# GenomicBreeding/GenomicBreedingModels.jl

Hardware: AMD Instinct MI355X
Metric: GRM+GBLUP genotype-cells/s (n x p) (higher is better)
Workload: dtype f64

## Files before the change

### genomicbreedingmodels.jl_amd/csrc/grm.hip

```cpp
#include <algorithm>
#include <atomic>
#include <cmath>
#include <cstdio>
#include <cstdlib>
#include <map>
#include <mutex>
#include <queue>
#include <tuple>
#include <vector>

#include "chol_device.h"

namespace gbm {

constexpr int BT = 128;
constexpr int BK = 16;
constexpr int WPS = 2;
constexpr int LROW = BT + 2;
constexpr int STAGE = 2 * BK * LROW;

__device__ __forceinline__ void tile_of(int64_t t, int64_t& ti, int64_t& tj) {
  int64_t r = (int64_t)((sqrt(8.0 * (double)t + 1.0) - 1.0) * 0.5);
  while ((r + 1) * (r + 2) / 2 <= t) r++;
  while (r * (r + 1) / 2 > t) r--;
  tj = r;
  ti = t - r * (r + 1) / 2;
}

enum SyrkMode { kSub = 0, kSplit = 1, kPersist = 2, kPersistFused = 3 };

struct TileOwner {
  int32_t rank = 0, nranks = 1;
  int64_t rhs_tile = -1;
  int64_t j_first = 0, ncols = 0;
  int32_t rhs = 0;
  int64_t ti0 = 0;
};

template <bool NEG>
__device__ __forceinline__ void tile_pass(const double* __restrict__ U, int64_t ldu, int64_t K, int64_t i0,
                                          int64_t j0, bool diag, bool active, int64_t kstep0, int64_t nsteps,
                                          double* lds, d4 (&acc)[4][4], int wave, int lane) {
  const int wm = wave >> 1, wn = wave & 1;
  auto stage_row = [&](int64_t kstep, int buf, int rr) {
    double* base = lds + buf * STAGE;
    const int r = wave * (BK / 4) + rr;
    const int64_t k = kstep * BK + r;
    double* la = base + r * LROW;
    double* lb = base + (BK + r) * LROW;
#ifdef GBM_SYRK_TIMING_NOLOAD
    if (k < K) {
    } else {
#else
    if (k < K) {
      const double* src = U + k * ldu;
      __builtin_amdgcn_global_load_lds((const void*)(src + i0 + lane * 2), (void*)la, 16, 0, 0);
      if (!diag) __builtin_amdgcn_global_load_lds((const void*)(src + j0 + lane * 2), (void*)lb, 16, 0, 0);
    } else {
#endif
      *reinterpret_cast<double2*>(la + lane * 2) = make_double2(0.0, 0.0);
      if (!diag) *reinterpret_cast<double2*>(lb + lane * 2) = make_double2(0.0, 0.0);
    }
  };
  const int frag_row = lane >> 4;
  const int frag_col = lane & 15;

  if (nsteps > 0) {
#pragma unroll
    for (int rr = 0; rr < BK / 4; rr++) stage_row(kstep0, 0, rr);
  }
  __syncthreads();
  for (int64_t st = 0; st < nsteps; st++) {
    const int buf = (int)(st & 1);
    if (st + 1 < nsteps) {
#pragma unroll
      for (int rr = 0; rr < BK / 4; rr++) stage_row(kstep0 + st + 1, buf ^ 1, rr);
    }
    const double* A = lds + buf * STAGE;
    const double* B = diag ? A : A + BK * LROW;
#pragma unroll
    for (int ks = 0; ks < BK / 4; ks++) {
      if (active) {
        const int kr = ks * 4 + frag_row;
        const double2 a01 = *reinterpret_cast<const double2*>(&A[kr * LROW + wm * 64 + 4 * frag_col]);
        const double2 a23 = *reinterpret_cast<const double2*>(&A[kr * LROW + wm * 64 + 4 * frag_col + 2]);
        const double2 b01 = *reinterpret_cast<const double2*>(&B[kr * LROW + wn * 64 + 4 * frag_col]);
        const double2 b23 = *reinterpret_cast<const double2*>(&B[kr * LROW + wn * 64 + 4 * frag_col + 2]);
        double af[4] = {a01.x, a01.y, a23.x, a23.y};
        const double bf[4] = {b01.x, b01.y, b23.x, b23.y};
        if constexpr (NEG) {
#pragma unroll
          for (int m = 0; m < 4; m++) af[m] = -af[m];
        }
        __builtin_amdgcn_s_setprio(1);
#pragma unroll
        for (int m = 0; m < 4; m++)
#pragma unroll
          for (int q = 0; q < 4; q++)
            acc[m][q] = __builtin_amdgcn_mfma_f64_16x16x4f64(af[m], bf[q], acc[m][q], 0, 0, 0);
        __builtin_amdgcn_s_setprio(0);
      }
    }
    __syncthreads();
  }
  __syncthreads();
}

constexpr int kMaxSlices = 32;
struct SliceBounds {
  int32_t n;
  int32_t b[kMaxSlices + 1];
  int32_t carry;
  int32_t er, et, erb, es, ekper;
  int64_t e0, eslab_off;
  int32_t accum = 0;
  int32_t fuse = 0;
};

template <int ET>
__device__ __forceinline__ void grm_edge_pass(const double* __restrict__ U, int64_t ldu, int64_t K,
                                              const SliceBounds& sb, int64_t e, double* __restrict__ part,
                                              int lane, int wave) {
  const int rb = (int)(e % sb.erb), ks = (int)(e / sb.erb);
  const int64_t k0 = (int64_t)ks * sb.ekper;
  const int64_t k1 = (k0 + sb.ekper < K) ? k0 + sb.ekper : K;
  const int64_t i0 = (int64_t)rb * 256 + wave * 64;
  const int fr = lane >> 4, fc = lane & 15;
  d4 acc[4][ET];
#pragma unroll
  for (int m = 0; m < 4; m++)
#pragma unroll
    for (int q = 0; q < ET; q++) acc[m][q] = (d4){0.0, 0.0, 0.0, 0.0};
  for (int64_t k = k0; k < k1; k += 16) {
    double a[4][4], b[4][ET];
#pragma unroll
    for (int st = 0; st < 4; st++) {
      const int64_t kk = k + st * 4 + fr;
      const bool kv = kk < k1;
      const double* row = U + kk * ldu;
#pragma unroll
      for (int m = 0; m < 4; m++) {
        const int64_t i = i0 + m * 16 + fc;
        a[st][m] = (kv && i < ldu) ? row[i] : 0.0;
      }
#pragma unroll
      for (int q = 0; q < ET; q++) b[st][q] = kv ? row[sb.e0 + q * 16 + fc] : 0.0;
    }
#pragma unroll
    for (int st = 0; st < 4; st++)
#pragma unroll
      for (int q = 0; q < ET; q++)
#pragma unroll
        for (int m = 0; m < 4; m++) acc[m][q] = __builtin_amdgcn_mfma_f64_16x16x4f64(a[st][m], b[st][q], acc[m][q], 0, 0, 0);
  }
  const int64_t rows = (int64_t)sb.erb * 256;
  constexpr int w = 16 * ET;
#pragma unroll
  for (int m = 0; m < 4; m++)
#pragma unroll
    for (int q = 0; q < ET; q++)
#pragma unroll
      for (int r = 0; r < 4; r++)
        part[((int64_t)ks * rows + i0 + m * 16 + fr + 4 * r) * w + q * 16 + fc] = acc[m][q][r];
}

template <int ET>
__global__ void __launch_bounds__(256, ET == 1 ? 4 : 1) grm_edge_kernel(const double* __restrict__ U, int64_t ldu, int64_t K,
                                                       SliceBounds sb, double* __restrict__ part) {
  grm_edge_pass<ET>(U, ldu, K, sb, blockIdx.x, part, threadIdx.x & 63, threadIdx.x >> 6);
}

__global__ void __launch_bounds__(256) grm_edge_reduce_kernel(const double* __restrict__ part, int64_t n,
                                                              SliceBounds sb, double* __restrict__ G, int64_t ldg,
                                                              int accum) {
  const int64_t idx = (int64_t)blockIdx.x * 256 + threadIdx.x;
  if (idx >= n * sb.er) return;
  const int64_t i = idx / sb.er;
  const int c = (int)(idx - i * sb.er);
  const int64_t rows = (int64_t)sb.erb * 256;
  const int w = 16 * sb.et;
  double acc = 0.0;
  for (int s = 0; s < sb.es; s++) acc += part[((int64_t)s * rows + i) * w + c];
  double* g = G + i * ldg + sb.e0 + c;
  *g = accum ? *g + acc : acc;
}

template <int MODE>
__global__ void __launch_bounds__(256, WPS)
syrk_kernel(const double* __restrict__ U, int64_t ldu, int64_t K, int64_t c0, int64_t lim,
            double* __restrict__ C, int64_t ldc, double* __restrict__ slab, int64_t ntiles, SliceBounds sb,
            double* __restrict__ Ld, double* __restrict__ Dinv, int32_t* __restrict__ info, int64_t fk0,
            TileOwner own) {
  constexpr int LDS_DOUBLES = (2 * STAGE > CNB * PS + CNB + 16) ? 2 * STAGE : CNB * PS + CNB + 16;
  __shared__ __attribute__((aligned(16))) double lds[LDS_DOUBLES];

  const int64_t wg = blockIdx.x;
  const int lane = threadIdx.x & 63;
  const int wave = __builtin_amdgcn_readfirstlane(threadIdx.x >> 6);
  const int wm = wave >> 1, wn = wave & 1;
  const int frag_row = lane >> 4, frag_col = lane & 15;
  const int64_t nst = (K + BK - 1) / BK;
  const int64_t rlim = c0 + lim;

  if constexpr (MODE == kSplit || MODE == kPersist || MODE == kPersistFused) {
    auto run_unit = [&](int sl, int64_t t) {
    int64_t ti, tj;
    tile_of(t, ti, tj);
    const bool diag = (ti == tj);
    const int64_t i0 = c0 + ti * BT, j0 = c0 + tj * BT;
    const bool active = (i0 + wm * 64 < rlim) && (j0 + wn * 64 < rlim) && !(diag && wm == 1 && wn == 0);
    d4 acc[4][4];
#pragma unroll
    for (int a = 0; a < 4; a++)
#pragma unroll
      for (int b = 0; b < 4; b++) acc[a][b] = (d4){0.0, 0.0, 0.0, 0.0};
    const int64_t ks0 = sb.b[sl];
    const int64_t ks1 = sb.b[sl + 1] < nst ? sb.b[sl + 1] : nst;
    tile_pass<false>(U, ldu, K, i0, j0, diag, active, ks0, ks1 > ks0 ? ks1 - ks0 : 0, lds, acc, wave, lane);
    if (MODE == kSplit && sb.carry && sb.n > 1) {
      int32_t* tflags = reinterpret_cast<int32_t*>(slab);
      double* out = C + i0 * ldc + j0 + (wm * 64 + 4 * frag_row) * ldc + wn * 64 + 4 * frag_col;
      if (sl > 0 || sb.accum) {
        if (sl > 0) {
          if (threadIdx.x == 0) wait_flag(&tflags[t], sl, tflags + ntiles);
          __syncthreads();
          __builtin_amdgcn_fence(__ATOMIC_ACQUIRE, "agent");
        }
        if (active) {
          double2 prev[4][4][2];
#pragma unroll
          for (int m = 0; m < 4; m++)
#pragma unroll
            for (int r = 0; r < 4; r++) {
              const double* o = out + (16 * r + m) * ldc;
              prev[m][r][0] = *reinterpret_cast<const double2*>(o);
              prev[m][r][1] = *reinterpret_cast<const double2*>(o + 2);
            }
#pragma unroll
          for (int m = 0; m < 4; m++)
#pragma unroll
            for (int r = 0; r < 4; r++) {
              acc[m][0][r] = prev[m][r][0].x + acc[m][0][r];
              acc[m][1][r] = prev[m][r][0].y + acc[m][1][r];
              acc[m][2][r] = prev[m][r][1].x + acc[m][2][r];
              acc[m][3][r] = prev[m][r][1].y + acc[m][3][r];
            }
        }
      }
      if (active) {
#pragma unroll
        for (int m = 0; m < 4; m++)
#pragma unroll
          for (int r = 0; r < 4; r++) {
            double* o = out + (16 * r + m) * ldc;
#pragma unroll
            for (int q = 0; q < 4; q++) st_agent(o + q, acc[m][q][r]);
          }
      }
      publish_flag(&tflags[t], sl + 1, threadIdx.x);
    } else if (MODE == kPersistFused && sb.n > 1) {
      const int64_t per = (int64_t)BT * BT;
      const int64_t eoff = (wm * 64 + 4 * frag_row) * BT + wn * 64 + 4 * frag_col;
      if (active) {
        double* out = slab + ((int64_t)sl * ntiles + t) * per + eoff;
#pragma unroll
        for (int m = 0; m < 4; m++)
#pragma unroll
          for (int r = 0; r < 4; r++) {
            double* o = out + (16 * r + m) * BT;
            *reinterpret_cast<double2*>(o) = make_double2(acc[m][0][r], acc[m][1][r]);
            *reinterpret_cast<double2*>(o + 2) = make_double2(acc[m][2][r], acc[m][3][r]);
          }
      }
      asm volatile("s_waitcnt vmcnt(0)" ::: "memory");
      __syncthreads();
      int* s_last = reinterpret_cast<int*>(lds);
      if (threadIdx.x == 0) {
        __builtin_amdgcn_fence(__ATOMIC_RELEASE, "agent");
        asm volatile("s_waitcnt vmcnt(0)" ::: "memory");
        const bool lt = __hip_atomic_fetch_add(&info[8 + t], 1, __ATOMIC_RELAXED, __HIP_MEMORY_SCOPE_AGENT) == sb.n - 1;
        if (lt) {
          __builtin_amdgcn_fence(__ATOMIC_ACQUIRE, "agent");
          asm volatile("s_waitcnt vmcnt(0)" ::: "memory");
        }
        *s_last = lt;
      }
      __syncthreads();
      const bool last = *s_last != 0;
      __syncthreads();
      if (last && active) {
        double* gout = C + (i0 + wm * 64 + 4 * frag_row) * ldc + j0 + wn * 64 + 4 * frag_col;
        const double* tbase = slab + t * per + eoff;
#pragma unroll 1
        for (int mr = 0; mr < 16; mr++) {
          const int m = mr & 3, r = mr >> 2;
          double2 v01 = make_double2(0.0, 0.0), v23 = make_double2(0.0, 0.0);
          for (int s2 = 0; s2 < sb.n; s2++) {
            const double* src = tbase + (int64_t)s2 * ntiles * per + (16 * r + m) * BT;
            const double2 x01 = *reinterpret_cast<const double2*>(src), x23 = *reinterpret_cast<const double2*>(src + 2);
            v01.x += x01.x;
            v01.y += x01.y;
            v23.x += x23.x;
            v23.y += x23.y;
          }
          double* g = gout + (16 * r + m) * ldc;
          if (sb.accum) {
            const double2 a01 = *reinterpret_cast<const double2*>(g), a23 = *reinterpret_cast<const double2*>(g + 2);
            v01 = make_double2(a01.x + v01.x, a01.y + v01.y);
            v23 = make_double2(a23.x + v23.x, a23.y + v23.y);
          }
          *reinterpret_cast<double2*>(g) = v01;
          *reinterpret_cast<double2*>(g + 2) = v23;
        }
      }
    } else if (active) {
      const int64_t ld = sb.n == 1 ? ldc : BT;
      double* out = (sb.n == 1 ? C + i0 * ldc + j0 : slab + ((int64_t)sl * ntiles + t) * (BT * BT)) +
                    (wm * 64 + 4 * frag_row) * ld + wn * 64 + 4 * frag_col;
#pragma unroll
      for (int m = 0; m < 4; m++)
#pragma unroll
        for (int r = 0; r < 4; r++) {
          double* o = out + (16 * r + m) * ld;
          *reinterpret_cast<double2*>(o) = make_double2(acc[m][0][r], acc[m][1][r]);
          *reinterpret_cast<double2*>(o + 2) = make_double2(acc[m][2][r], acc[m][3][r]);
        }
    }
    };
    const int64_t T8 = (ntiles + 7) & ~(int64_t)7;
    if constexpr (MODE == kPersist || MODE == kPersistFused) {
      __shared__ int64_t s_unit;
      int32_t* ctr = info;
      const int xcc = (int)(__builtin_amdgcn_s_getreg((20 << 0) | (0 << 6) | (31 << 11)) & 7);
      const int64_t per = T8 >> 3;
      int q = xcc;
      for (int tries = 0; tries < 8;) {
        const int64_t qt0 = q * per;
        const int64_t qt1 = qt0 + per < ntiles ? qt0 + per : ntiles;
        const int64_t nq = qt1 > qt0 ? qt1 - qt0 : 0;
        if (threadIdx.x == 0) s_unit = atomicAdd(&ctr[q], 1);
        __syncthreads();
        const int64_t u = s_unit;
        __syncthreads();
        if (u >= nq * sb.n) {
          q = (q + 1) & 7;
          tries++;
          continue;
        }
        const int sl = (int)(u / nq);
        run_unit(sl, qt0 + (u - (int64_t)sl * nq));
      }
      return;
    } else {
      const int sl = (int)(wg / T8);
      const int64_t u = wg - (int64_t)sl * T8;
      const int64_t t = (u & 7) * (T8 >> 3) + (u >> 3);
      if (t >= ntiles) return;
      run_unit(sl, t);
    }
    return;
  } else {
    int64_t ti, tj;
    if (own.nranks > 1) {
      const int64_t c = blockIdx.y;
      const int64_t J = c < own.ncols ? own.j_first + c * own.nranks : own.rhs_tile;
      tj = J - c0 / BT;
      ti = own.ti0 + blockIdx.x;
      if (ti > tj) return;
    } else {
      tile_of(wg, ti, tj);
    }
    const bool diag = (ti == tj);
    const int64_t i0 = c0 + ti * BT, j0 = c0 + tj * BT;
    const bool active = (i0 + wm * 64 < rlim) && (j0 + wn * 64 < rlim) && !(diag && wm == 1 && wn == 0);
    d4 acc[4][4];
    const int64_t col0 = j0 + wn * 64 + 4 * frag_col;
#pragma unroll
    for (int m = 0; m < 4; m++)
#pragma unroll
      for (int r = 0; r < 4; r++) {
        const int64_t row = i0 + wm * 64 + 4 * frag_row + 16 * r + m;
        double2 c01 = make_double2(0.0, 0.0), c23 = make_double2(0.0, 0.0);
        if (active && row < rlim && col0 < rlim) {
          c01 = *reinterpret_cast<const double2*>(C + row * ldc + col0);
          c23 = *reinterpret_cast<const double2*>(C + row * ldc + col0 + 2);
        }
        acc[m][0][r] = c01.x;
        acc[m][1][r] = c01.y;
        acc[m][2][r] = c23.x;
        acc[m][3][r] = c23.y;
      }
    tile_pass<true>(U, ldu, K, i0, j0, diag, active, 0, nst, lds, acc, wave, lane);
    const bool factor_next = fk0 >= 0 && wg == 0;
    if (!active && !factor_next) return;
#pragma unroll
    for (int m = 0; m < 4; m++)
#pragma unroll
      for (int r = 0; r < 4; r++) {
        const int64_t row = i0 + wm * 64 + 4 * frag_row + 16 * r + m;
        if (active && row < rlim && col0 < rlim) {
          *reinterpret_cast<double2*>(C + row * ldc + col0) = make_double2(acc[m][0][r], acc[m][1][r]);
          *reinterpret_cast<double2*>(C + row * ldc + col0 + 2) = make_double2(acc[m][2][r], acc[m][3][r]);
        }
      }
    if (factor_next) {
      double* Us = lds;
      double* rinv = lds + CNB * PS;
      if (wave == 0) {
#pragma unroll
        for (int m = 0; m < 4; m++)
#pragma unroll
          for (int q = 0; q < 4; q++)
#pragma unroll
            for (int r = 0; r < 4; r++) Us[(4 * frag_row + 16 * r + m) * PS + 4 * frag_col + q] = acc[m][q][r];
      }
      __syncthreads();
      const int bad = factor_diag_block(Us, rinv, threadIdx.x);
      if (threadIdx.x == 0 && bad >= 0) atomicCAS(info, 0, (int32_t)(fk0 + bad + 1));
      store_factor(Us, rinv, Ld + fk0 * CNB, Dinv + (fk0 / 16) * 256, threadIdx.x);
    }
  }
}

#ifndef GBM_GRM_RED_NT
#define GBM_GRM_RED_NT 1
#endif
__global__ void __launch_bounds__(256) grm_slab_reduce_kernel(const double* __restrict__ slab, int64_t ntiles,
                                                              int nslices, double* __restrict__ G, int64_t ldg,
                                                              int accum) {
  const int64_t t = blockIdx.x;
  int64_t ti, tj;
  tile_of(t, ti, tj);
  const int64_t per = (int64_t)BT * BT;
  for (int e = threadIdx.x * 2; e < BT * BT; e += 256 * 2) {
    double2 acc = make_double2(0.0, 0.0);
    for (int sl = 0; sl < nslices; sl++) {
#if GBM_GRM_RED_NT
      typedef double d2v __attribute__((ext_vector_type(2)));
      const d2v v = __builtin_nontemporal_load(reinterpret_cast<const d2v*>(slab + ((int64_t)sl * ntiles + t) * per + e));
#else
      const double2 v = *reinterpret_cast<const double2*>(slab + ((int64_t)sl * ntiles + t) * per + e);
#endif
      acc.x += v.x;
      acc.y += v.y;
    }
    const int row = e / BT, col = e % BT;
    double2* g = reinterpret_cast<double2*>(G + (ti * BT + row) * ldg + tj * BT + col);
    if (accum) {
      const double2 old = *g;
      acc.x = old.x + acc.x;
      acc.y = old.y + acc.y;
    }
    *g = acc;
  }
}

static int resident_wgs() {
  int dev = 0, cus = 256;
  if (hipGetDevice(&dev) == hipSuccess) {
    int v = 0;
    if (hipDeviceGetAttribute(&v, hipDeviceAttributeMultiprocessorCount, dev) == hipSuccess && v > 0) cus = v;
  }
  return cus * WPS;
}

struct GrmTuning {
  int carry = -1;
  bool edge = true;
  bool persist = true;
  bool edge_concurrent = true;
  bool fuse = false;
  std::vector<double> split;
};

static GrmTuning grm_tuning() {
  GrmTuning t;
  auto flag = [](const char* name, bool dflt) {
    const char* e = ::gbm::knob(name);
    return e ? atoi(e) != 0 : dflt;
  };
  if (const char* e = ::gbm::knob("GBM_GRM_CARRY")) t.carry = atoi(e) != 0 ? 1 : 0;
  t.edge = flag("GBM_GRM_EDGE", true);
  t.persist = flag("GBM_GRM_PERSIST", true);
  t.edge_concurrent = flag("GBM_GRM_EDGE_CONCURRENT", true);
  t.fuse = flag("GBM_GRM_FUSED", false);
  if (const char* ov = ::gbm::knob("GBM_GRM_SPLIT")) {
    for (const char* q = ov; *q;) {
      char* end = nullptr;
      const double x = strtod(q, &end);
      if (end == q) break;
      if (x > 0) t.split.push_back(x);
      q = (*end == ',') ? end + 1 : end;
    }
    if ((int)t.split.size() > kMaxSlices) t.split.clear();
  }
  return t;
}

struct GrmPlan {
  int64_t ntiles, nst, tile_elems;
  SliceBounds sb;
  int64_t main_doubles, edge_doubles;
  bool persist, edge_concurrent;
};

static double simulate_split(const std::vector<int64_t>& sizes, const std::vector<double>& cost, int64_t R,
                             double tile_bytes, double stage_s, bool carry) {
  std::vector<double> speed(R);
  uint64_t h = 0x9E3779B97F4A7C15ull;
  for (int64_t k = 0; k < R; k++) {
    h = h * 6364136223846793005ull + 1442695040888963407ull;
    speed[k] = 1.0 + 0.035 * (((double)(h >> 11) / 9007199254740992.0) * 2.0 - 1.0);
  }
  std::priority_queue<std::pair<double, int64_t>, std::vector<std::pair<double, int64_t>>, std::greater<>> slots;
  for (int64_t k = 0; k < R; k++) slots.push({0.0, k});
  double makespan = 0.0;
  for (size_t s = 0; s < sizes.size(); s++)
    for (double c : cost) {
      auto [f, k] = slots.top();
      slots.pop();
      f += (double)sizes[s] * c * ((s == 0 && f > 0.0) ? 1.10 : 1.0) / speed[k];
      if (carry && s > 0) f += 0.5;
      if (f > makespan) makespan = f;
      slots.push({f, k});
    }
  const double reduce_stages =
      carry ? 0.0 : (double)sizes.size() * (double)cost.size() * tile_bytes / 4e12 / stage_s;
  return makespan + reduce_stages;
}

static GrmPlan plan(int64_t n, int64_t p) {
  const GrmTuning tune = grm_tuning();
  GrmPlan g;
  const int64_t nt_all = npad_of(n) / BT;
  const int64_t r_last = n - (nt_all - 1) * BT;
  const bool edge = tune.edge && nt_all >= 8 && r_last <= 64;
  const int64_t nt = edge ? nt_all - 1 : nt_all;
  g.nst = (p + BK - 1) / BK;
  std::vector<double> cost;
  const int64_t R = resident_wgs();
  for (int64_t tj = 0; tj < nt; tj++)
    for (int64_t ti = 0; ti <= tj; ti++) cost.push_back(ti == tj ? 0.93 : 1.0);
  g.ntiles = nt * (nt + 1) / 2;
  g.tile_elems = (int64_t)BT * BT;
  auto finish = [&](GrmPlan& gp) {
    gp.main_doubles = gp.sb.n == 1 ? 0
                      : gp.sb.carry ? (gp.ntiles + 1 + 1) / 2 + 1
                                    : (int64_t)gp.sb.n * gp.ntiles * gp.tile_elems;
    gp.sb.er = 0;
    gp.sb.et = gp.sb.erb = gp.sb.es = gp.sb.ekper = 0;
    gp.sb.e0 = gp.sb.eslab_off = 0;
    gp.edge_doubles = 0;
    if (edge) {
      gp.sb.e0 = nt * BT;
      gp.sb.er = (int32_t)r_last;
      gp.sb.et = (int32_t)((r_last + 15) / 16);
      gp.sb.erb = (int32_t)((n + 255) / 256);
      const int64_t es_want = std::max<int64_t>(1, std::min<int64_t>((2048 + gp.sb.erb - 1) / gp.sb.erb, (p + 255) / 256));
      gp.sb.ekper = (int32_t)(((p + es_want - 1) / es_want + 15) / 16 * 16);
      gp.sb.es = (int32_t)((p + gp.sb.ekper - 1) / gp.sb.ekper);
      gp.sb.eslab_off = gp.main_doubles;
      gp.edge_doubles = (int64_t)gp.sb.es * gp.sb.erb * 256 * 16 * gp.sb.et;
    }
    gp.persist = tune.persist && !gp.sb.carry;
    gp.sb.fuse = (gp.persist && gp.sb.n > 1 && tune.fuse) ? 1 : 0;
    gp.edge_concurrent = gp.sb.er > 0 && gp.persist && tune.edge_concurrent;
  };
  static std::mutex mu;
  static std::map<std::tuple<int64_t, int64_t, int64_t, int, std::vector<double>>, SliceBounds> cache;
  std::lock_guard<std::mutex> lock(mu);
  auto key = std::make_tuple(nt, g.nst, R, tune.carry, tune.split);
  auto it = cache.find(key);
  if (it != cache.end()) {
    g.sb = it->second;
    finish(g);
    return g;
  }
  const int64_t minc = 16;
  const bool big = g.ntiles > 2048;
  const double stage_s = 3.9e-6;
  double best = 1e300;
  auto choose = [&](bool carry) {
    std::vector<std::vector<int64_t>> cands;
    const int max_uniform = big ? 3 : (carry ? kMaxSlices : 8);
    for (int S = 1; S <= max_uniform; S++) {
      if (S > 1 && g.nst / S < minc) break;
      std::vector<int64_t> v;
      for (int i = 0; i < S; i++) v.push_back((g.nst * (i + 1)) / S - (g.nst * i) / S);
      cands.push_back(v);
    }
    for (double f = big ? 0.60 : 0.40; f < 0.90; f += big ? 0.10 : 0.05)
      for (double r : {0.3, 0.4, 0.5, 0.6, 0.7}) {
        if (big && r != 0.5) continue;
        std::vector<int64_t> v;
        int64_t first = (int64_t)(f * (double)g.nst);
        if (first < minc || g.nst - first < minc) continue;
        v.push_back(first);
        int64_t rem = g.nst - first;
        while (rem > 0) {
          int64_t c = (int64_t)std::ceil(r * (double)rem);
          if (c < minc) c = minc;
          if (rem - c < minc || (int)v.size() == (carry ? kMaxSlices : 12) - 1) c = rem;
          v.push_back(c);
          rem -= c;
        }
        cands.push_back(v);
      }
    if (!tune.split.empty()) {
      double tot = 0;
      for (double x : tune.split) tot += x;
      cands.clear();
      std::vector<int64_t> v;
      int64_t acc = 0;
      double cum = 0;
      for (size_t i = 0; i < tune.split.size(); i++) {
        cum += tune.split[i];
        const int64_t e = (i + 1 == tune.split.size()) ? g.nst : (int64_t)std::llround(cum / tot * (double)g.nst);
        if (e > acc) v.push_back(e - acc);
        acc = e > acc ? e : acc;
      }
      cands.push_back(v);
    }
    std::vector<int64_t> bv{g.nst};
    best = 1e300;
    for (const auto& v : cands) {
      const double m = simulate_split(v, cost, R, (double)g.tile_elems * 8.0, stage_s, carry);
      if (m < best * 0.999) {
        best = m;
        bv = v;
      }
    }
    return bv;
  };
  int carry_mode = tune.carry;
  std::vector<int64_t> bestv = choose(carry_mode == 1);
  if (carry_mode < 0 && bestv.size() > 1 &&
      (double)bestv.size() * (double)g.ntiles * (double)g.tile_elems * 8.0 > 4.0 * 1073741824.0) {
    carry_mode = 1;
    bestv = choose(true);
  }
  g.sb.carry = (carry_mode == 1 && bestv.size() > 1) ? 1 : 0;
  g.sb.n = (int32_t)bestv.size();
  g.sb.b[0] = 0;
  for (int i = 0; i < g.sb.n; i++) g.sb.b[i + 1] = g.sb.b[i] + (int32_t)bestv[i];
  cache.emplace(key, g.sb);
  finish(g);
  return g;
}

constexpr int P64 = 80;
template <bool PIPE>
__global__ void __launch_bounds__(256, 2)
syrk64_sub_kernel(const double* __restrict__ U, int64_t ldu, int64_t c0, int64_t lim, double* __restrict__ C,
                  int64_t ldc, double* Ld, double* Dinv, int32_t* __restrict__ info,
                  int64_t fk0, int rowonly, int kchunks, ColKeep keep) {
  __shared__ __attribute__((aligned(16))) double As[64 * P64];
  __shared__ __attribute__((aligned(16))) double Bs[64 * P64];
  int64_t ti = 0, tj = blockIdx.x;
  if (!rowonly) tile_of(blockIdx.x, ti, tj);
  const bool diag = ti == tj;
  const int64_t i0 = c0 + ti * 64, j0 = c0 + tj * 64;
  if (rowonly && !col_kept(keep, j0)) return;
  const int tid = threadIdx.x, lane = tid & 63, wave = tid >> 6;
  const int wm = wave >> 1, wn = wave & 1;
  const int fr = lane >> 4, fc = lane & 15;
  const int64_t rlim = c0 + lim;
  const bool active = (i0 + wm * 32 < rlim) && (j0 + wn * 32 < rlim);
  d4 acc[2][2];
  if (active) {
#pragma unroll
    for (int m = 0; m < 2; m++)
#pragma unroll
      for (int q = 0; q < 2; q++)
#pragma unroll
        for (int r = 0; r < 4; r++) {
          const int64_t row = i0 + wm * 32 + m * 16 + fr + 4 * r;
          const int64_t col = j0 + wn * 32 + q * 16 + fc;
          acc[m][q][r] = (row < rlim && col < rlim) ? C[row * ldc + col] : 0.0;
        }
  }
  const double* B = Bs;
  const int lrow = tid >> 5, lcol = 2 * (tid & 31);
  typedef double d16 __attribute__((ext_vector_type(16)));
  d16 va, vb;
  auto load_chunk = [&](int c) {
    const double* sa = U + (c * 64 + lrow) * ldu + i0 + lcol;
    const double* sb = U + (c * 64 + lrow) * ldu + j0 + lcol;
#pragma unroll
    for (int e = 0; e < 8; e++) {
      const double2 x = *reinterpret_cast<const double2*>(sa + 8 * e * ldu);
      const double2 y = *reinterpret_cast<const double2*>(sb + 8 * e * ldu);
      va[2 * e] = x.x;
      va[2 * e + 1] = x.y;
      vb[2 * e] = y.x;
      vb[2 * e + 1] = y.y;
    }
  };
  load_chunk(0);
  for (int c = 0; c < kchunks; c++) {
    if (c > 0) __syncthreads();
#pragma unroll
    for (int e = 0; e < 8; e++) {
      *reinterpret_cast<double2*>(&As[(lrow + 8 * e) * P64 + lcol]) = make_double2(va[2 * e], va[2 * e + 1]);
      *reinterpret_cast<double2*>(&Bs[(lrow + 8 * e) * P64 + lcol]) = make_double2(vb[2 * e], vb[2 * e + 1]);
    }
    __syncthreads();
    if (PIPE && c + 1 < kchunks) load_chunk(c + 1);
    if (active) {
#pragma unroll
      for (int ks = 0; ks < 16; ks++) {
        double af[2], bf[2];
#pragma unroll
        for (int m = 0; m < 2; m++) af[m] = -As[(ks * 4 + fr) * P64 + wm * 32 + m * 16 + fc];
#pragma unroll
        for (int q = 0; q < 2; q++) bf[q] = B[(ks * 4 + fr) * P64 + wn * 32 + q * 16 + fc];
#pragma unroll
        for (int m = 0; m < 2; m++)
#pragma unroll
          for (int q = 0; q < 2; q++)
            acc[m][q] = __builtin_amdgcn_mfma_f64_16x16x4f64(af[m], bf[q], acc[m][q], 0, 0, 0);
      }
    }
    if (!PIPE && c + 1 < kchunks) load_chunk(c + 1);
  }
  const bool factor_next = fk0 >= 0 && blockIdx.x == 0;
  if (!active && !factor_next) return;
#pragma unroll
  for (int m = 0; m < 2; m++)
#pragma unroll
    for (int q = 0; q < 2; q++)
#pragma unroll
      for (int r = 0; r < 4; r++) {
        const int64_t row = i0 + wm * 32 + m * 16 + fr + 4 * r;
        const int64_t col = j0 + wn * 32 + q * 16 + fc;
        if (active && row < rlim && col < rlim) C[row * ldc + col] = acc[m][q][r];
      }
  if (factor_next) {
    __syncthreads();
    double* Us = As;
    double* rinv = Bs;
#pragma unroll
    for (int m = 0; m < 2; m++)
#pragma unroll
      for (int q = 0; q < 2; q++)
#pragma unroll
        for (int r = 0; r < 4; r++) Us[(wm * 32 + m * 16 + fr + 4 * r) * PS + wn * 32 + q * 16 + fc] = acc[m][q][r];
    __syncthreads();
    const int bad = factor_diag_block(Us, rinv, tid);
    if (tid == 0 && bad >= 0) atomicCAS(info, 0, (int32_t)(fk0 + bad + 1));
    store_factor(Us, rinv, Ld + fk0 * CNB, Dinv + (fk0 / 16) * 256, tid);
  }
}

static std::atomic<int64_t> g_small_lim{2048};
void chol_refresh_tuning() {
  const char* e = ::gbm::knob("GBM_UPD64_LIM");
  g_small_lim.store(e ? (int64_t)atoll(e) : (int64_t)2048, std::memory_order_relaxed);
}
int64_t chol_small_lim() { return g_small_lim.load(std::memory_order_relaxed); }

int launch_chol_row_update(double* G, int64_t ldg, int64_t k0, int kch, int64_t gdim, double* Ld, double* Dinv,
                           int32_t* info, hipStream_t s, ColKeep keep) {
  const int64_t k1 = k0 + 64 * (int64_t)kch;
  const int64_t lim = gdim - k1;
  if (kch > 1)
    syrk64_sub_kernel<true><<<(unsigned)(lim / 64), 256, 0, s>>>(G + k0 * ldg, ldg, k1, lim, G, ldg, Ld, Dinv, info, k1,
                                                             1, kch, keep);
  else
    syrk64_sub_kernel<false><<<(unsigned)(lim / 64), 256, 0, s>>>(G + k0 * ldg, ldg, k1, lim, G, ldg, Ld, Dinv, info, k1,
                                                              1, kch, keep);
  GBM_LAUNCH_CHECK();
  return GBM_OK;
}

int launch_chol_update(double* G, int64_t ldg, int64_t k0, int64_t nb, int64_t gdim, double* Ld, double* Dinv,
                       int32_t* info, int64_t next_k0, int rank, int nranks, hipStream_t s, int64_t col_lo,
                       int64_t col_hi, int64_t row_lo, int64_t row_hi) {
  const int64_t k1 = k0 + nb;
  const int64_t lim = gdim - k1;
  if (lim <= 0) return GBM_OK;
  TileOwner own;
  if (nranks > 1) {
    if ((k1 % BT) != 0 || nb == 64 || (col_lo % BT) != 0 || (row_lo % BT) != 0)
      return fail(GBM_E_ARG, "distributed Cholesky update: panel groups, column and row ranges on 128-column tiles");
    own.rank = rank;
    own.nranks = nranks;
    own.rhs_tile = (gdim - kRhsRows) / BT;
    const int64_t jlo = std::max(k1, col_lo) / BT;
    const int64_t jhi = col_hi >= gdim ? own.rhs_tile : std::min((col_hi + BT - 1) / BT, own.rhs_tile);
    own.j_first = jlo + ((rank - jlo) % nranks + nranks) % nranks;
    own.ncols = own.j_first < jhi ? (jhi - own.j_first + nranks - 1) / nranks : 0;
    own.rhs = col_hi >= gdim ? 1 : 0;
    if (own.ncols + own.rhs == 0) return GBM_OK;
    own.ti0 = (std::max(row_lo, k1) - k1) / BT;
    const int64_t ti1 = (std::min(row_hi, gdim) - k1 + BT - 1) / BT;
    if (ti1 <= own.ti0) return GBM_OK;
    const int64_t m = ti1 - own.ti0;
    syrk_kernel<kSub><<<dim3((unsigned)m, (unsigned)(own.ncols + own.rhs)), 256, 0, s>>>(
        G + k0 * ldg, ldg, nb, k1, lim, G, ldg, nullptr, 0, SliceBounds{}, Ld, Dinv, info, -1, own);
    GBM_LAUNCH_CHECK();
    return GBM_OK;
  }
  if (nb == 64 && lim <= chol_small_lim()) {
    const int64_t m = (lim + 63) / 64;
    syrk64_sub_kernel<false><<<(unsigned)(m * (m + 1) / 2), 256, 0, s>>>(G + k0 * ldg, ldg, k1, lim, G, ldg, Ld, Dinv, info,
                                                                  next_k0, 0, (int)(nb / 64), ColKeep{});
    GBM_LAUNCH_CHECK();
    return GBM_OK;
  }
  const int64_t m = (lim + BT - 1) / BT;
  const int64_t ntiles = m * (m + 1) / 2;
  syrk_kernel<kSub><<<(unsigned)ntiles, 256, 0, s>>>(G + k0 * ldg, ldg, nb, k1, lim, G, ldg, nullptr, ntiles, SliceBounds{}, Ld,
                                                     Dinv, info, next_k0, own);
  GBM_LAUNCH_CHECK();
  return GBM_OK;
}

struct AuxStream {
  hipStream_t s = nullptr;
  hipEvent_t fork = nullptr, join = nullptr;
  ~AuxStream() {
    if (fork) (void)hipEventDestroy(fork);
    if (join) (void)hipEventDestroy(join);
  }
};
static int aux_stream(hipStream_t caller, AuxStream& a, bool* usable) {
  *usable = false;
  int dev = 0;
  GBM_HIP_TRY(hipGetDevice(&dev));
  if (caller) {
    int sdev = -1;
    if (hipStreamGetDevice(caller, &sdev) != hipSuccess) {
      (void)hipGetLastError();
      return GBM_OK;
    }
    if (sdev != dev) return GBM_OK;
  }
  static std::mutex mu;
  static std::map<int, hipStream_t> streams;
  {
    std::lock_guard<std::mutex> lock(mu);
    hipStream_t& hs = streams[dev];
    if (!hs) GBM_HIP_TRY(hipStreamCreateWithFlags(&hs, hipStreamNonBlocking));
    a.s = hs;
  }
  GBM_HIP_TRY(hipEventCreateWithFlags(&a.fork, hipEventDisableTiming));
  GBM_HIP_TRY(hipEventCreateWithFlags(&a.join, hipEventDisableTiming));
  *usable = true;
  return GBM_OK;
}

static int64_t grm_counter_doubles(const GrmPlan& g) { return 4 + (g.sb.fuse ? (g.ntiles + 1) / 2 : 0); }
int64_t grm_workspace_bytes(int64_t n, int64_t p) {
  const GrmPlan g = plan(n, p);
  return (g.main_doubles + g.edge_doubles + grm_counter_doubles(g)) * (int64_t)sizeof(double);
}

static int check_grm_args(const double* Zt, int64_t ldz, int64_t p, int64_t n, double* G, int64_t ldg) {
  const int64_t npad = npad_of(n);
  if (!Zt || !G || p < 1 || n < 1 || ldz < npad || ldg < npad || (ldz & 1) || (ldg & 1))
    return fail(GBM_E_ARG, "gbm_dev_grm: bad arguments (need ldz, ldg >= npad(n), both even)");
  if (((uintptr_t)Zt & 15) != 0 || ((uintptr_t)G & 15) != 0)
    return fail(GBM_E_ARG, "gbm_dev_grm: Zt and G must be 16-byte aligned");
  return GBM_OK;
}

int launch_grm_syrk(const double* Zt, int64_t ldz, int64_t p, int64_t n, double* G, int64_t ldg, void* ws,
                    int64_t ws_bytes, hipStream_t s, int accum = 0) {
  int rc = check_grm_args(Zt, ldz, p, n, G, ldg);
  if (rc != GBM_OK) return rc;
  const GrmPlan g = plan(n, p);
  SliceBounds sb = g.sb;
  sb.accum = accum;
  const int64_t need = (g.main_doubles + g.edge_doubles + grm_counter_doubles(g)) * (int64_t)sizeof(double);
  if (need > 0 && (!ws || ws_bytes < need))
    return fail(GBM_E_ARG, "gbm_dev_grm: workspace too small (" + std::to_string(ws_bytes) + " < " +
                               std::to_string(need) + ")");
  const unsigned grid = (unsigned)(g.sb.n * ((g.ntiles + 7) & ~(int64_t)7));
  if (g.sb.carry) GBM_HIP_TRY(hipMemsetAsync(ws, 0, (size_t)(g.ntiles + 1) * sizeof(int32_t), s));
  int32_t* ctr = reinterpret_cast<int32_t*>((double*)ws + g.main_doubles + g.edge_doubles);
  const int64_t lim = g.sb.er > 0 ? g.sb.e0 : n;
  AuxStream aux;
  AuxStream* ax = nullptr;
  if (g.edge_concurrent) {
    bool usable = false;
    rc = aux_stream(s, aux, &usable);
    if (rc != GBM_OK) return rc;
    if (usable) {
      ax = &aux;
      GBM_HIP_TRY(hipEventRecord(ax->fork, s));
      GBM_HIP_TRY(hipStreamWaitEvent(ax->s, ax->fork, 0));
    }
  }
  if (g.persist) {
    GBM_HIP_TRY(hipMemsetAsync(ctr, 0, (size_t)(8 + (g.sb.fuse ? g.ntiles : 0)) * sizeof(int32_t), s));
    const int64_t units = (int64_t)g.sb.n * g.ntiles;
    const unsigned pgrid = (unsigned)(units < resident_wgs() ? units : resident_wgs());
    if (g.sb.fuse)
      syrk_kernel<kPersistFused><<<pgrid, 256, 0, s>>>(Zt, ldz, p, 0, lim, G, ldg, (double*)ws, g.ntiles, sb, nullptr,
                                                       nullptr, ctr, -1, TileOwner{});
    else
      syrk_kernel<kPersist><<<pgrid, 256, 0, s>>>(Zt, ldz, p, 0, lim, G, ldg, (double*)ws, g.ntiles, sb, nullptr,
                                                  nullptr, ctr, -1, TileOwner{});
  } else {
    syrk_kernel<kSplit><<<grid, 256, 0, s>>>(Zt, ldz, p, 0, lim, G, ldg, (double*)ws, g.ntiles, sb, nullptr, nullptr,
                                             nullptr, -1, TileOwner{});
  }
  GBM_LAUNCH_CHECK();
  if (g.sb.er > 0) {
    const hipStream_t es = ax ? ax->s : s;
    const unsigned eg = (unsigned)((int64_t)g.sb.erb * g.sb.es);
    double* part = (double*)ws + g.sb.eslab_off;
    switch (g.sb.et) {
      case 1: grm_edge_kernel<1><<<eg, 256, 0, es>>>(Zt, ldz, p, g.sb, part); break;
      case 2: grm_edge_kernel<2><<<eg, 256, 0, es>>>(Zt, ldz, p, g.sb, part); break;
      case 3: grm_edge_kernel<3><<<eg, 256, 0, es>>>(Zt, ldz, p, g.sb, part); break;
      default: grm_edge_kernel<4><<<eg, 256, 0, es>>>(Zt, ldz, p, g.sb, part); break;
    }
    GBM_LAUNCH_CHECK();
    if (g.edge_concurrent) {
      grm_edge_reduce_kernel<<<(unsigned)((n * g.sb.er + 255) / 256), 256, 0, es>>>(part, n, g.sb, G, ldg, accum);
      GBM_LAUNCH_CHECK();
    }
    if (ax) {
      GBM_HIP_TRY(hipEventRecord(ax->join, ax->s));
      GBM_HIP_TRY(hipStreamWaitEvent(s, ax->join, 0));
    }
  }
  return GBM_OK;
}

int launch_grm_reduce(int64_t n, int64_t p, double* G, int64_t ldg, const void* ws, hipStream_t s, int accum = 0,
                      int32_t* err_out = nullptr) {
  const GrmPlan g = plan(n, p);
  if (g.sb.n == 1 && g.sb.er == 0) return GBM_OK;
  if (!ws) return fail(GBM_E_ARG, "gbm_dev_grm_reduce: workspace required");
  if (g.sb.er > 0 && !g.edge_concurrent) {
    grm_edge_reduce_kernel<<<(unsigned)((n * g.sb.er + 255) / 256), 256, 0, s>>>((const double*)ws + g.sb.eslab_off, n,
                                                                                 g.sb, G, ldg, accum);
    GBM_LAUNCH_CHECK();
  }
  if (g.sb.n == 1 || g.sb.fuse) return GBM_OK;
  if (g.sb.carry && err_out) {
    GBM_HIP_TRY(hipMemcpyAsync(err_out, (const int32_t*)ws + g.ntiles, sizeof(int32_t), hipMemcpyDeviceToDevice, s));
    return GBM_OK;
  }
  if (g.sb.carry) {
    int32_t err = 0;
    GBM_HIP_TRY(hipMemcpyAsync(&err, (const int32_t*)ws + g.ntiles, sizeof(int32_t), hipMemcpyDeviceToHost, s));
    GBM_HIP_TRY(hipStreamSynchronize(s));
    if (err < 0)
      return fail(GBM_E_HIP, "GRM in-order carry accumulation: an inter-workgroup wait timed out (G is invalid)");
    return GBM_OK;
  }
  grm_slab_reduce_kernel<<<(unsigned)g.ntiles, 256, 0, s>>>((const double*)ws, g.ntiles, g.sb.n, G, ldg, accum);
  GBM_LAUNCH_CHECK();
  return GBM_OK;
}

int launch_grm(const double* Zt, int64_t ldz, int64_t p, int64_t n, double* G, int64_t ldg, void* ws,
               int64_t ws_bytes, hipStream_t s, int accum, int32_t* err_out) {
  if (accum && !grm_can_accumulate(n, p)) return fail(GBM_E_ARG, "GRM: accumulation needs the slab split");
  int rc = launch_grm_syrk(Zt, ldz, p, n, G, ldg, ws, ws_bytes, s, accum);
  if (rc != GBM_OK) return rc;
  return launch_grm_reduce(n, p, G, ldg, ws, s, accum, err_out);
}

bool grm_can_accumulate(int64_t n, int64_t p) {
  const GrmPlan g = plan(n, p);
  return g.sb.n > 1;
}

}

namespace gbm {
__global__ void __launch_bounds__(256) grm_pack_kernel(const double* __restrict__ G, int64_t ldg,
                                                       double* __restrict__ packed, int unpack) {
  const int64_t t = blockIdx.x;
  int64_t ti, tj;
  tile_of(t, ti, tj);
  double* pt = packed + t * (int64_t)(BT * BT);
  for (int e = threadIdx.x * 2; e < BT * BT; e += 512) {
    const int r = e / BT, c = e % BT;
    double* g = const_cast<double*>(G) + (ti * BT + r) * ldg + tj * BT + c;
    if (unpack)
      *reinterpret_cast<double2*>(g) = *reinterpret_cast<const double2*>(pt + e);
    else
      *reinterpret_cast<double2*>(pt + e) = *reinterpret_cast<const double2*>(g);
  }
}
}

extern "C" int64_t gbm_dev_grm_packed_size(int64_t n) {
  const int64_t nt = gbm::npad_of(n) / gbm::BT;
  return nt * (nt + 1) / 2 * gbm::BT * gbm::BT;
}

extern "C" int gbm_dev_grm_pack(const double* G, int64_t ldg, int64_t n, double* packed, void* stream) {
  if (!G || !packed || n < 1 || ldg < gbm::npad_of(n) || (ldg & 1)) return gbm::fail(GBM_E_ARG, "gbm_dev_grm_pack: bad arguments");
  const int64_t nt = gbm::npad_of(n) / gbm::BT;
  gbm::grm_pack_kernel<<<(unsigned)(nt * (nt + 1) / 2), 256, 0, (hipStream_t)stream>>>(G, ldg, packed, 0);
  GBM_LAUNCH_CHECK();
  return GBM_OK;
}

extern "C" int gbm_dev_grm_unpack(const double* packed, int64_t n, double* G, int64_t ldg, void* stream) {
  if (!G || !packed || n < 1 || ldg < gbm::npad_of(n) || (ldg & 1)) return gbm::fail(GBM_E_ARG, "gbm_dev_grm_unpack: bad arguments");
  const int64_t nt = gbm::npad_of(n) / gbm::BT;
  gbm::grm_pack_kernel<<<(unsigned)(nt * (nt + 1) / 2), 256, 0, (hipStream_t)stream>>>(G, ldg, const_cast<double*>(packed), 1);
  GBM_LAUNCH_CHECK();
  return GBM_OK;
}

extern "C" int64_t gbm_dev_grm_workspace(int64_t n, int64_t p) { return gbm::grm_workspace_bytes(n, p); }

extern "C" int gbm_dev_grm(const double* Zt, int64_t ldz, int64_t p, int64_t n, double* G, int64_t ldg,
                           void* workspace, int64_t ws_bytes, void* stream) {
  return gbm::launch_grm(Zt, ldz, p, n, G, ldg, workspace, ws_bytes, (hipStream_t)stream);
}

extern "C" int gbm_dev_grm_accumulate(const double* Zt, int64_t ldz, int64_t p, int64_t n, double* G, int64_t ldg,
                                      void* workspace, int64_t ws_bytes, void* stream) {
  if (!gbm::grm_can_accumulate(n, p))
    return gbm::fail(GBM_E_ARG, "gbm_dev_grm_accumulate: this (n, p) plans a single loci range (gbm_dev_grm_slices == 1); "
                                "use more loci per call");
  return gbm::launch_grm(Zt, ldz, p, n, G, ldg, workspace, ws_bytes, (hipStream_t)stream, 1);
}

extern "C" int gbm_dev_grm_syrk(const double* Zt, int64_t ldz, int64_t p, int64_t n, double* G, int64_t ldg,
                                void* workspace, int64_t ws_bytes, void* stream) {
  return gbm::launch_grm_syrk(Zt, ldz, p, n, G, ldg, workspace, ws_bytes, (hipStream_t)stream);
}

extern "C" int gbm_dev_grm_reduce(int64_t n, int64_t p, double* G, int64_t ldg, const void* workspace, void* stream) {
  if (!G || n < 1 || p < 1 || ldg < gbm::npad_of(n)) return gbm::fail(GBM_E_ARG, "gbm_dev_grm_reduce: bad arguments");
  return gbm::launch_grm_reduce(n, p, G, ldg, workspace, (hipStream_t)stream);
}

extern "C" int gbm_dev_grm_slices(int64_t n, int64_t p) {
  return gbm::plan(n, p).sb.n;
}

namespace gbm {
__global__ void __launch_bounds__(256) add_inplace_kernel(double* __restrict__ a, const double* __restrict__ b,
                                                          int64_t n) {
  for (int64_t i = ((int64_t)blockIdx.x * 256 + threadIdx.x) * 2; i < n; i += (int64_t)gridDim.x * 512) {
    if (i + 1 < n) {
      double2 x = *reinterpret_cast<const double2*>(a + i);
      const double2 y = *reinterpret_cast<const double2*>(b + i);
      x.x += y.x;
      x.y += y.y;
      *reinterpret_cast<double2*>(a + i) = x;
    } else {
      a[i] += b[i];
    }
  }
}

int launch_add_inplace(double* a, const double* b, int64_t n, hipStream_t s) {
  if (n <= 0) return GBM_OK;
  const int64_t want = (n + 511) / 512;
  add_inplace_kernel<<<(unsigned)(want < 8192 ? want : 8192), 256, 0, s>>>(a, b, n);
  GBM_LAUNCH_CHECK();
  return GBM_OK;
}

__global__ void __launch_bounds__(256) grm_export_kernel(const double* __restrict__ G, int64_t ldg, int64_t n,
                                                         double inv_q, double* __restrict__ out, int64_t ldo) {
  const int64_t i = blockIdx.x;
  for (int64_t j = threadIdx.x; j < n; j += 256)
    out[i * ldo + j] = inv_q * (j >= i ? G[i * ldg + j] : G[j * ldg + i]);
}

int launch_grm_export(const double* G, int64_t ldg, int64_t n, double inv_q, double* out, int64_t ldo, hipStream_t s) {
  grm_export_kernel<<<(unsigned)n, 256, 0, s>>>(G, ldg, n, inv_q, out, ldo);
  GBM_LAUNCH_CHECK();
  return GBM_OK;
}
}
```

Baseline: 11.85 billion.

## Add specialized symmetric diagonal-tile kernel that computes only upper-triangle blocks

Adds a dedicated path for diagonal 128x128 tiles in which each of the four waves computes a balanced set of upper-triangular 16x16 blocks (9 MFMA accumulators per wave), instead of the generic 2x2 wave layout that idles one wave. Each wave stages a quarter of the K rows into LDS and stores its blocks directly to C or the slice slab. The scheduler's cost model gives diagonal tiles a lower weight (0.66) so slice balancing reflects the cheaper work. It is gated by a knob, is skipped for partial tiles, carry mode and fused mode, and relies on the lower triangle of diagonal tiles not being needed.

```diff
diff --git a/genomicbreedingmodels.jl_amd/csrc/grm.hip b/genomicbreedingmodels.jl_amd/csrc/grm.hip
--- a/genomicbreedingmodels.jl_amd/csrc/grm.hip
+++ b/genomicbreedingmodels.jl_amd/csrc/grm.hip
@@ -106,6 +106,84 @@
   __syncthreads();
 }
 
+template <int W>
+__device__ __forceinline__ void diag_step(const double* __restrict__ Ak, d4 (&acc)[9]) {
+  double x[8];
+#pragma unroll
+  for (int X = W; X < 8; X++) x[X] = Ak[16 * X];
+  __builtin_amdgcn_s_setprio(1);
+#pragma unroll
+  for (int J = W; J < 8; J++) acc[J - W] = __builtin_amdgcn_mfma_f64_16x16x4f64(x[W], x[J], acc[J - W], 0, 0, 0);
+#pragma unroll
+  for (int J = 7 - W; J < 8; J++)
+    acc[1 + J] = __builtin_amdgcn_mfma_f64_16x16x4f64(x[7 - W], x[J], acc[1 + J], 0, 0, 0);
+  __builtin_amdgcn_s_setprio(0);
+}
+
+template <int W>
+__device__ __forceinline__ void diag_store(double* __restrict__ out, int64_t ld, const d4 (&acc)[9]) {
+  int64_t row0 = 16 * W * ld, row1 = 16 * (7 - W) * ld, step = 4 * ld;
+  asm volatile("" : "+s"(row0), "+s"(row1), "+s"(step));
+  double* o = out + row0;
+#pragma unroll
+  for (int r = 0; r < 4; r++, o += step)
+#pragma unroll
+    for (int J = W; J < 8; J++) o[16 * J] = acc[J - W][r];
+  o = out + row1;
+#pragma unroll
+  for (int r = 0; r < 4; r++, o += step)
+#pragma unroll
+    for (int J = 7 - W; J < 8; J++) o[16 * J] = acc[1 + J][r];
+}
+
+template <int W>
+__device__ __forceinline__ void diag_tile_wave(const double* __restrict__ U, int64_t ldu, int64_t K, int64_t i0,
+                                          int64_t kstep0, int64_t nsteps, double* lds, double* __restrict__ out,
+                                          int64_t ld, int lane) {
+  auto stage_row = [&](int64_t kstep, int buf, int rr) {
+    const int r = W * (BK / 4) + rr;
+    const int64_t k = kstep * BK + r;
+    double* la = lds + buf * STAGE + r * LROW;
+    if (k < K)
+      __builtin_amdgcn_global_load_lds((const void*)(U + k * ldu + i0 + lane * 2), (void*)la, 16, 0, 0);
+    else
+      *reinterpret_cast<double2*>(la + lane * 2) = make_double2(0.0, 0.0);
+  };
+  d4 acc[9];
+#pragma unroll
+  for (int a = 0; a < 9; a++) acc[a] = (d4){0.0, 0.0, 0.0, 0.0};
+  if (nsteps > 0) {
+#pragma unroll
+    for (int rr = 0; rr < BK / 4; rr++) stage_row(kstep0, 0, rr);
+  }
+  __syncthreads();
+  for (int64_t st = 0; st < nsteps; st++) {
+    const int buf = (int)(st & 1);
+    if (st + 1 < nsteps) {
+#pragma unroll
+      for (int rr = 0; rr < BK / 4; rr++) stage_row(kstep0 + st + 1, buf ^ 1, rr);
+    }
+    const double* A = lds + buf * STAGE + (lane >> 4) * LROW + (lane & 15);
+#pragma unroll
+    for (int ks = 0; ks < BK / 4; ks++) diag_step<W>(A + ks * 4 * LROW, acc);
+    __syncthreads();
+  }
+  __syncthreads();
+  diag_store<W>(out + (lane >> 4) * ld + (lane & 15), ld, acc);
+}
+
+__device__ __forceinline__ void diag_tile(const double* __restrict__ U, int64_t ldu, int64_t K, int64_t i0,
+                                          int64_t kstep0, int64_t nsteps, double* lds, double* __restrict__ out,
+                                          int64_t ld, int wave, int lane) {
+  asm volatile("" : "+v"(lane));
+  switch (wave) {
+    case 0: diag_tile_wave<0>(U, ldu, K, i0, kstep0, nsteps, lds, out, ld, lane); break;
+    case 1: diag_tile_wave<1>(U, ldu, K, i0, kstep0, nsteps, lds, out, ld, lane); break;
+    case 2: diag_tile_wave<2>(U, ldu, K, i0, kstep0, nsteps, lds, out, ld, lane); break;
+    default: diag_tile_wave<3>(U, ldu, K, i0, kstep0, nsteps, lds, out, ld, lane); break;
+  }
+}
+
 constexpr int kMaxSlices = 32;
 struct SliceBounds {
   int32_t n;
@@ -115,6 +193,7 @@
   int64_t e0, eslab_off;
   int32_t accum = 0;
   int32_t fuse = 0;
+  int32_t diag = 0;
 };
 
 template <int ET>
@@ -209,13 +288,21 @@
     const bool diag = (ti == tj);
     const int64_t i0 = c0 + ti * BT, j0 = c0 + tj * BT;
     const bool active = (i0 + wm * 64 < rlim) && (j0 + wn * 64 < rlim) && !(diag && wm == 1 && wn == 0);
-    d4 acc[4][4];
-#pragma unroll
-    for (int a = 0; a < 4; a++)
-#pragma unroll
-      for (int b = 0; b < 4; b++) acc[a][b] = (d4){0.0, 0.0, 0.0, 0.0};
     const int64_t ks0 = sb.b[sl];
     const int64_t ks1 = sb.b[sl + 1] < nst ? sb.b[sl + 1] : nst;
+    if constexpr (MODE != kPersistFused) {
+      if (diag && sb.diag && i0 + BT <= rlim && !(MODE == kSplit && sb.carry && sb.n > 1)) {
+        diag_tile(U, ldu, K, i0, ks0, ks1 > ks0 ? ks1 - ks0 : 0, lds,
+                  sb.n == 1 ? C + i0 * ldc + j0 : slab + ((int64_t)sl * ntiles + t) * (BT * BT), sb.n == 1 ? ldc : BT,
+                  wave, lane);
+        return;
+      }
+    }
+    d4 acc[4][4];
+#pragma unroll
+    for (int a = 0; a < 4; a++)
+#pragma unroll
+      for (int b = 0; b < 4; b++) acc[a][b] = (d4){0.0, 0.0, 0.0, 0.0};
     tile_pass<false>(U, ldu, K, i0, j0, diag, active, ks0, ks1 > ks0 ? ks1 - ks0 : 0, lds, acc, wave, lane);
     if (MODE == kSplit && sb.carry && sb.n > 1) {
       int32_t* tflags = reinterpret_cast<int32_t*>(slab);
@@ -470,6 +557,8 @@
   bool persist = true;
   bool edge_concurrent = true;
   bool fuse = false;
+  bool diag = true;
+  double diag_cost = 0.66;
   std::vector<double> split;
 };
 
@@ -484,6 +573,12 @@
   t.persist = flag("GBM_GRM_PERSIST", true);
   t.edge_concurrent = flag("GBM_GRM_EDGE_CONCURRENT", true);
   t.fuse = flag("GBM_GRM_FUSED", false);
+  t.diag = flag("GBM_GRM_DIAG", true);
+  if (const char* e = ::gbm::knob("GBM_GRM_DIAG_COST")) {
+    const double c = atof(e);
+    if (c > 0.0 && c <= 1.0) t.diag_cost = c;
+  }
+  if (!t.diag) t.diag_cost = 0.93;
   if (const char* ov = ::gbm::knob("GBM_GRM_SPLIT")) {
     for (const char* q = ov; *q;) {
       char* end = nullptr;
@@ -540,7 +635,7 @@
   std::vector<double> cost;
   const int64_t R = resident_wgs();
   for (int64_t tj = 0; tj < nt; tj++)
-    for (int64_t ti = 0; ti <= tj; ti++) cost.push_back(ti == tj ? 0.93 : 1.0);
+    for (int64_t ti = 0; ti <= tj; ti++) cost.push_back(ti == tj ? tune.diag_cost : 1.0);
   g.ntiles = nt * (nt + 1) / 2;
   g.tile_elems = (int64_t)BT * BT;
   auto finish = [&](GrmPlan& gp) {
@@ -564,12 +659,13 @@
     }
     gp.persist = tune.persist && !gp.sb.carry;
     gp.sb.fuse = (gp.persist && gp.sb.n > 1 && tune.fuse) ? 1 : 0;
+    gp.sb.diag = tune.diag ? 1 : 0;
     gp.edge_concurrent = gp.sb.er > 0 && gp.persist && tune.edge_concurrent;
   };
   static std::mutex mu;
-  static std::map<std::tuple<int64_t, int64_t, int64_t, int, std::vector<double>>, SliceBounds> cache;
+  static std::map<std::tuple<int64_t, int64_t, int64_t, int, std::vector<double>, bool, double>, SliceBounds> cache;
   std::lock_guard<std::mutex> lock(mu);
-  auto key = std::make_tuple(nt, g.nst, R, tune.carry, tune.split);
+  auto key = std::make_tuple(nt, g.nst, R, tune.carry, tune.split, tune.diag, tune.diag_cost);
   auto it = cache.find(key);
   if (it != cache.end()) {
     g.sb = it->second;
```

New measurement: 12.01 billion, median of 6. 1.01x the previous value.
